# lkeegan/blockCG

Hardware: AMD Instinct MI355X
Metric: SBCGrQ lattice-site iterations/sec (iterations/sec x global volume), fp64 (higher is better)
Workload: dtype f64; 1 GPU; SBCGrQ V=64x64x64x64 (64x64x64x64 per GPU), m=16, 4 shifts, mass=0.001, fixed-work (eps=0); m=16, transport=none, half_volume_solves=False, memory_ladder_rung=whole tmp

## Files before the change

### blockcg_amd/csrc/capi_context.hip

```cpp
#include "capi_internal.hpp"

namespace bcg_impl {

std::string g_create_error;

void resolve_profile(bcg_context* c) {
  for (auto& kv : c->prof) {
    for (auto& pr : kv.second.pending) {
      float ms = 0.f;
      if (hipEventElapsedTime(&ms, pr.first, pr.second) == hipSuccess) {
        kv.second.ms += ms;
        kv.second.count += 1;
      }
      c->event_pool.push_back(pr.first);
      c->event_pool.push_back(pr.second);
    }
    kv.second.pending.clear();
  }
}

int stream_sync(bcg_context* c) {
  HIP_TRY(c, hipStreamSynchronize(c->stream));
  c->mat_in_flight = 0;
  if (c->profiling) resolve_profile(c);
// ... 272 lines not shown

}

using namespace bcg_impl;

extern "C" {

const char* bcg_last_error(const bcg_context* ctx) { return ctx ? ctx->err.c_str() : g_create_error.c_str(); }

int bcg_context_create(bcg_context** out, int device, void* stream, int ndim, const int* global_dims, const int* grid,
                       const int* coords) {
  if (!out || !global_dims || ndim < 1 || ndim > 4) {
    g_create_error = "bcg_context_create: bad arguments";
    return BCG_ERR_INVALID;
  }
  int ndev = 0;
  if (hipGetDeviceCount(&ndev) != hipSuccess || ndev <= 0 || device < 0 || device >= ndev) {
    g_create_error = "bcg_context_create: no usable HIP device (this library has no CPU fallback)";
    return BCG_ERR_NO_DEVICE;
  }
  hipDeviceProp_t prop;
  if (hipGetDeviceProperties(&prop, device) != hipSuccess) {
    g_create_error = "bcg_context_create: hipGetDeviceProperties failed";
    return BCG_ERR_NO_DEVICE;
  }
  if (std::strncmp(prop.gcnArchName, "gfx950", 6) != 0) {
    g_create_error = std::string("bcg_context_create: device is not gfx950 (MI355X): ") + prop.gcnArchName;
    return BCG_ERR_NO_DEVICE;
  }
  if (hipSetDevice(device) != hipSuccess) {
    g_create_error = "bcg_context_create: hipSetDevice failed";
    return BCG_ERR_HIP;
  }
  bcg_context* c = new bcg_context();
  c->device = device;
  c->ndim = ndim;
  int64_t V = 1;
  int64_t ghost = 0;
  for (int mu = 0; mu < 4; ++mu) {
    c->gdims[mu] = mu < ndim ? global_dims[mu] : 1;
    c->grid[mu] = (mu < ndim && grid) ? grid[mu] : 1;
    c->coords[mu] = (mu < ndim && coords) ? coords[mu] : 0;
    if (c->gdims[mu] < 1 || c->grid[mu] < 1 || c->gdims[mu] % c->grid[mu] != 0 || c->coords[mu] < 0 ||
        c->coords[mu] >= c->grid[mu]) {
      g_create_error = "bcg_context_create: lattice extents must be positive multiples of the process grid";
      delete c;
      return BCG_ERR_INVALID;
    }
    c->lat.L[mu] = c->gdims[mu] / c->grid[mu];
    c->lat.origin[mu] = c->coords[mu] * c->lat.L[mu];
    c->lat.split[mu] = c->grid[mu] > 1 ? 1 : 0;
    c->lat.stride[mu] = V;
    V *= c->lat.L[mu];
    if (c->lat.split[mu]) c->distributed = true;
  }
  c->lat.ndim = ndim;
  c->lat.V = V;
  for (int mu = 0; mu < 4; ++mu) {
    c->lat.face_sites[mu] = V / c->lat.L[mu];
    c->lat.ghost_off[mu][0] = c->lat.ghost_off[mu][1] = 0;
    if (c->lat.split[mu]) {
      c->lat.ghost_off[mu][0] = ghost;
      c->lat.ghost_off[mu][1] = ghost + c->lat.face_sites[mu];
      ghost += 2 * c->lat.face_sites[mu];
    }
  }
  c->ghost_sites = ghost;
  if (const char* e = std::getenv("BCG_ROW_BLOCKS_B")) c->row_blocks_B = std::atoi(e);
  if (const char* e = std::getenv("BCG_ROW_BLOCKS_C")) c->row_blocks_C = std::atoi(e);
  if (const char* e = std::getenv("BCG_ROW_BATCHED")) c->row_batched = std::atoi(e) != 0;
  if (const char* e = std::getenv("BCG_HOP_FACTORED")) c->hop_factored = std::atoi(e) != 0;
  if (const char* e = std::getenv("BCG_HOP_WALK")) c->hop_tune.patch_walk = std::atoi(e) != 0;
  if (const char* e = std::getenv("BCG_HOP_BLOCKS")) c->hop_tune.blocks = std::atoi(e);
  if (const char* e = std::getenv("BCG_HOP_BLOCKS_OVERLAP")) c->hop_tune.blocks_overlap = std::atoi(e);
  if (const char* e = std::getenv("BCG_HOP_SUPER")) c->hop_tune.super_patch = std::atoi(e);
  if (const char* e = std::getenv("BCG_HOP_SYNC")) c->hop_tune.sync.window = std::atoi(e);
  if (const char* e = std::getenv("BCG_HOP_SYNC_LIMIT")) c->hop_tune.sync.limit_ticks = std::atoi(e);
  if (const char* e = std::getenv("BCG_HOP_COLUMN")) c->hop_tune.sync.column_walk = std::atoi(e) != 0;
  if (const char* e = std::getenv("BCG_HOP_BUNDLE")) c->hop_tune.sync.bundle_walk = std::atoi(e);
  if (const char* e = std::getenv("BCG_HOP_BUNDLE_SYNC")) c->hop_tune.sync.bundle_window = std::atoi(e);
  if (const char* e = std::getenv("BCG_LAZY_Q")) c->lazy_q = std::atoi(e);
  if (const char* e = std::getenv("BCG_PAIR_SHIFTS")) c->pair_shifts = std::atoi(e);
  if (const char* e = std::getenv("BCG_DEFER_X0")) c->defer_x0 = std::atoi(e) != 0;
  if (const char* e = std::getenv("BCG_DEBUG_X0_COND_LIMIT")) c->x0_cond_limit = std::atof(e);
  if (const char* e = std::getenv("BCG_RING_CHUNK")) c->ring_chunk_override = std::atoi(e);
  if (const char* e = std::getenv("BCG_DEBUG_FIELD_BUDGET")) c->debug_field_budget = static_cast<size_t>(std::atoll(e));
  if (const char* e = std::getenv("BCG_DEBUG_FAIL_ITER")) c->debug_fail_iter = std::atoi(e);
  if (const char* e = std::getenv("BCG_RING_OVERLAP")) c->ring_overlap = std::atoi(e) != 0;
  if (const char* e = std::getenv("BCG_HALF_CHUNK_FORCE")) c->half_chunk_force = std::atoi(e) != 0;
  if (const char* e = std::getenv("BCG_HALF_CHUNK")) c->half_chunk_override = std::atoi(e);
  if (const char* e = std::getenv("BCG_FORCE_TILE_CLASSES")) c->force_tile_classes = std::atoi(e) != 0;
  if (const char* e = std::getenv("BCG_HOP_PATCH")) std::sscanf(e, "%d,%d,%d", &c->hop_tune.patch[0], &c->hop_tune.patch[1], &c->hop_tune.patch[2]);
  if (stream) {
    c->stream = static_cast<hipStream_t>(stream);
  } else {
    if (hipStreamCreateWithFlags(&c->stream, hipStreamNonBlocking) != hipSuccess) {
      g_create_error = "bcg_context_create: hipStreamCreate failed";
      delete c;
      return BCG_ERR_HIP;
    }
    c->own_stream = true;
  }
  *out = c;
  return BCG_OK;
}

int bcg_context_destroy(bcg_context* c) {
  DeviceScope on_device(c);
  if (!c) return BCG_OK;
  (void)hipSetDevice(c->device);
  (void)hipStreamSynchronize(c->stream);
  for (auto& kv : c->tmp_field) {
    (void)hipFree(kv.second->base);
    delete kv.second;
  }
  for (auto& kv : c->tmp_ring_buf)
    if (kv.second) (void)hipFree(kv.second);
  for (auto& kv : c->boundary_tiles)
    if (kv.second.first) (void)hipFree(kv.second.first);
  if (c->halo_send) (void)hipFree(c->halo_send);
  if (c->halo_recv) (void)hipFree(c->halo_recv);
  if (c->halo_save) (void)hipFree(c->halo_save);
  if (c->partials) (void)hipFree(c->partials);
  if (c->hop_tune.sync.counters) (void)hipFree(c->hop_tune.sync.counters);
  if (c->dev_mats) (void)hipFree(c->dev_mats);
  if (c->pin_mats) (void)hipHostFree(c->pin_mats);
  if (c->dev_gram) (void)hipFree(c->dev_gram);
  if (c->fold_tickets) (void)hipFree(c->fold_tickets);
  if (c->pin_gram) (void)hipHostFree(c->pin_gram);
  if (c->dev_basis) (void)hipFree(c->dev_basis);
  if (c->pin_basis) (void)hipHostFree(c->pin_basis);
  if (c->basis_uploaded) (void)hipEventDestroy(c->basis_uploaded);
  if (c->dev_rotate) (void)hipFree(c->dev_rotate);
  if (c->pin_rotate) (void)hipHostFree(c->pin_rotate);
  if (c->rotate_uploaded) (void)hipEventDestroy(c->rotate_uploaded);
  if (c->staging) (void)hipFree(c->staging);
  for (int k = 0; k < 2; ++k) {
    if (c->xfer_stream[k]) (void)hipStreamSynchronize(c->xfer_stream[k]);
    if (c->xfer_dev[k]) (void)hipFree(c->xfer_dev[k]);
    if (c->xfer_pin[k]) (void)hipHostFree(c->xfer_pin[k]);
    if (c->xfer_done[k]) (void)hipEventDestroy(c->xfer_done[k]);
    if (c->xfer_stream[k]) (void)hipStreamDestroy(c->xfer_stream[k]);
    c->xfer_dev[k] = nullptr;
    c->xfer_pin[k] = nullptr;
    c->xfer_done[k] = nullptr;
    c->xfer_stream[k] = nullptr;
  }
  for (auto& kv : c->prof)
    for (auto& pr : kv.second.pending) {
      (void)hipEventDestroy(pr.first);
      (void)hipEventDestroy(pr.second);
    }
  for (hipEvent_t ev : c->event_pool) (void)hipEventDestroy(ev);
  if (c->own_stream) (void)hipStreamDestroy(c->stream);
  delete c;
  return BCG_OK;
}

int bcg_context_set_comm(bcg_context* c, const bcg_comm* comm) {
  if (!c) return BCG_ERR_INVALID;
  if (comm) {
    c->comm = *comm;
    c->have_comm = true;
  } else {
    c->have_comm = false;
  }
// ... 391 lines not shown
```

### blockcg_amd/csrc/capi_solvers.hip

```cpp
#include "capi_internal.hpp"

namespace bcg_impl {

int phase_A(bcg_context* c, const bcg_gauge* g, double mass, double sigma0, bcg_field* T, const bcg_field* P, CMat& G) {
  int nb = 0;
  bool folded = false, self = false;
  BCG_TRY(apply_shifted(c, g, mass, sigma0, T, P, &nb, &folded, &self));
  if (nb > 0) {
    BCG_TRY(finish_gram(c, P->m, nb, G, true, folded));
    c->phaseA_gram_raw = CMat(P->m, c->pin_gram);
    if (self)
      for (int i = 0; i < P->m; ++i) G(i, i) = G(i, i).real();
    c->phaseA_gram = G;
    return BCG_OK;
  }
  BCG_TRY(gram(c, P, T, G));
  c->phaseA_gram = G;
  c->phaseA_gram_raw = CMat();
  return BCG_OK;
}

int rmul(bcg_context* c, bcg_field* y, const bcg_field* x, const CMat& M, double b, bcg::RmulMode mode, const char* name);
bool lazy_q_width(const bcg_context* c, int m) {
  return c->lazy_q && fast_rows(c, m) && fast_rmul(c, m) && (m == 8 || m == 16 || (m == 32 && c->lazy_q > 1));
}

int phase_B(bcg_context* c, bcg_field* Q, const bcg_field* T, const CMat& alpha, CMat& G2, const CMat* rinv_prev = nullptr,
            bcg_field* Qout = nullptr) {
  const int m = Q->m;
  if (!fast_rows(c, m)) {
    if (Qout) BCG_FAIL(c, BCG_ERR_INVALID, "phase B: a separate output needs the fused kernel");
    BCG_TRY(rmul(c, Q, T, -alpha, 0.0, bcg::RMUL_ADD, "block_axpy"));
    return gram(c, Q, Q, G2);
  }
  const CMat na = -alpha;
  const CMat* two[2] = {&na, rinv_prev};
  const double2* Md;
  BCG_TRY(upload_mats(c, m, two, rinv_prev ? 2 : 1, &Md));
  int nb;
  {
    ProfScope ps(c, "phaseB", row_bytes(Q, 3), product_flops(Q, rinv_prev ? 3 : 2));
    nb = bcg::launch_phaseB(c->stream, m, rows_of(Q), Q->d, T->d, Md, c->partials, c->row_blocks_B, c->row_batched,
                            bcg::GramFold{c->dev_gram, c->fold_tickets},
                            rinv_prev ? Md + static_cast<size_t>(m) * m : nullptr, Qout ? Qout->d : nullptr);
  }
  BCG_TRY(check_launch(c, "phaseB"));
  return finish_gram(c, m, nb, G2, true, true);
}

int trisolve(bcg_context* c, bcg_field* y, const CMat& R);
int phase_C(bcg_context* c, bcg_field* Q, const CMat& rho, bcg_field* const* X, bcg_field* const* P, int n,
            const std::vector<CMat>& A, const std::vector<CMat>& Bm, CMat* rinv_out = nullptr, bcg_field* Y = nullptr) {
  const int m = Q->m;
  if (!fast_rmul(c, m)) {
    BCG_TRY(trisolve(c, Q, rho));
    for (int s = 0; s < n; ++s) {
      BCG_TRY(rmul(c, Y ? Y : X[s], P[s], A[s], 0.0, bcg::RMUL_ADD, "block_axpy"));
      BCG_TRY(rmul(c, P[s], Q, Bm[s], 1.0, bcg::RMUL_XPAY, "block_xpay"));
    }
    return BCG_OK;
  }
  const CMat Rinv = bcg::upper_triangular_inverse(rho);
  if (rinv_out) *rinv_out = Rinv;
  for (int s0 = 0, first = 1, per = 0; first || s0 < n; s0 += per, first = 0) {
    per = bcg::phaseC_max_shifts(m, first != 0);
    const int ns = std::min(per, n - s0);
    std::vector<const CMat*> mats;
    mats.push_back(&Rinv);
    double2* Xp[8];
    double2* Pp[8];
    for (int k = 0; k < ns; ++k) {
      mats.push_back(&A[s0 + k]);
      mats.push_back(&Bm[s0 + k]);
      Xp[k] = Y ? nullptr : X[s0 + k]->d;
      Pp[k] = P[s0 + k]->d;
    }
    const double2* Md;
    BCG_TRY(upload_mats(c, m, mats.data(), static_cast<int>(mats.size()), &Md));
    {
      ProfScope ps(c, Y ? "phaseC_sum" : "phaseC", row_bytes(Q, (first && !rinv_out ? 2 : 1) + (Y ? 2 * ns + (ns > 0 ? 2 : 0) : 4 * ns)),
                   product_flops(Q, (rinv_out || first ? 1 : 0) + 2 * ns));
      bcg::launch_phaseC(c->stream, m, rows_of(Q), Q->d, Xp, Pp, ns, Md, rinv_out ? 2 : first, c->row_blocks_C, Y ? Y->d : nullptr);
    }
    BCG_TRY(check_launch(c, "phaseC"));
  }
  return BCG_OK;
}

bool x0_may_wait(const bcg_context* c, int m) {
  return c->defer_x0 && lazy_q_width(c, m) && (m == 8 || m == 16) && !capacity_path(c, m);
}
int pair_shifts_depth(const bcg_context* c, int m, int n_shifts) {
  if (c->pair_shifts < 2 || !fast_rows(c, m) || !fast_rmul(c, m)) return 1;
  if (!lazy_q_width(c, m) && m != 32) return 1;
  if (m == 32 && lazy_q_width(c, m)) return 1;
  int d = std::min(c->pair_shifts, capacity_path(c, m) ? 2 : 4);
  while (d >= 2 && !bcg::phaseC_multi_fits(m, d, n_shifts)) --d;
  if (n_shifts < 2 && (d < 3 || !x0_may_wait(c, m))) return 1;
  return d;
}

struct DeferredIteration {
  bcg_field* Q = nullptr;
  CMat rinv;
  int n_active = 0;
  std::vector<CMat> A, B;
  bool x0_deferred = false;
  CMat A0, R0;
  bool x0_backward = false;
};

struct DeferredX0 {
  std::vector<CMat> mats;
};
DeferredX0 compose_x0(const std::vector<DeferredIteration>& pend) {
  DeferredX0 out;
  const int n = static_cast<int>(pend.size());
  if (n == 0 || !pend[0].x0_deferred || pend[0].x0_backward) return out;
  const int m = pend[0].A0.dim();
  for (int k = -1; k + 1 < n; ++k) {
    CMat sum(m), chain = CMat::identity(m);
    for (int i = k + 1; i < n; ++i) {
      sum = sum + chain * pend[i].A0;
      chain = chain * pend[i].R0;
    }
    out.mats.push_back(sum);
  }
  return out;
}

int phase_C_multi(bcg_context* c, const std::vector<DeferredIteration>& pend, bcg_field* Qnew, const CMat& rho_new,
                  bcg_field* const* X, bcg_field* const* P, const CMat& A0, const CMat& B0, int n_active_new,
                  const std::vector<CMat>& Anew, const std::vector<CMat>& Bnew, CMat* rinv_out, bool lazy,
                  const CMat* flush_rinv = nullptr, const bcg_field* p0_first = nullptr, bcg_field* Y = nullptr) {
  const int m = Qnew->m, ns = static_cast<int>(pend.size()) + 1;
  const CMat rinv_new = flush_rinv ? *flush_rinv : (lazy ? bcg::upper_triangular_inverse(rho_new) : CMat());
  const double2* Qd[4];
  for (int j = 0; j + 1 < ns; ++j) Qd[j] = pend[j].Q->d;
  Qd[ns - 1] = Qnew->d;
  struct Entry {
    int shift, first, last;
    std::vector<const CMat*> mats;
  };
  std::vector<Entry> entries;
  if (flush_rinv) {
  } else if (lazy) {
    entries.push_back(Entry{0, ns - 1, ns, {&A0, &B0}});
  } else {
    const std::vector<CMat> a0(1, A0), b0(1, B0);
    BCG_TRY(phase_C(c, Qnew, rho_new, X, P, 1, a0, b0, nullptr, Y));
  }
  const int n_first = ns > 1 ? pend[0].n_active : n_active_new;
  for (int s = 1; s < n_first; ++s) {
    Entry e{s, 0, 0, {}};
    for (int j = 0; j < ns; ++j) {
      const bool on = s < (j + 1 < ns ? pend[j].n_active : n_active_new);
      if (!on) break;
      e.mats.push_back(j + 1 < ns ? &pend[j].A[s] : &Anew[s]);
      e.mats.push_back(j + 1 < ns ? &pend[j].B[s] : &Bnew[s]);
      ++e.last;
    }
    entries.push_back(e);
  }
  DeferredX0 x0 = (p0_first && lazy && !flush_rinv) ? compose_x0(pend) : DeferredX0();
  CMat A0_back;
  if (!p0_first && lazy && !flush_rinv && ns == 2 && pend[0].x0_deferred && pend[0].x0_backward) {
    const CMat M = pend[0].rinv.adjoint() * pend[0].A0;
    A0_back = A0 + M;
    entries[0].mats[0] = &A0_back;
    x0.mats.push_back(CMat(m));
    x0.mats.push_back(-M);
  }
  const int xacc = static_cast<int>(x0.mats.size());
  if (xacc > 0) {
    for (const CMat& M : x0.mats) entries[0].mats.push_back(&M);
  }
  static const char* const names[5] = {"", "", "phaseC_multi2", "phaseC_multi3", "phaseC_multi4"};
  static const char* const sum_names[5] = {"", "", "phaseC_multi2_sum", "phaseC_multi3_sum", "phaseC_multi4_sum"};
  for (size_t e0 = 0; e0 < entries.size();) {
    const bool with_x0 = xacc > 0 && e0 == 0;
    int n = 0;
    for (int room = bcg::phaseC_multi_capacity(m) - (lazy ? ns : 0); e0 + n < entries.size() && n < 8; ++n) {
      room -= static_cast<int>(entries[e0 + n].mats.size());
      if (room < 0) break;
    }
    if (n == 0) BCG_FAIL(c, BCG_ERR_UNSUPPORTED, "phase C: the matrices of one entry do not fit a launch");
    std::vector<const CMat*> mats;
    if (lazy) {
      for (int j = 0; j + 1 < ns; ++j) mats.push_back(&pend[j].rinv);
      mats.push_back(&rinv_new);
    }
    double2* Xp[8];
    double2* Pp[8];
    int first[8], last[8];
    double products = lazy ? ns : 0;
    for (int k = 0; k < n; ++k) {
      const Entry& e = entries[e0 + k];
      Xp[k] = Y ? nullptr : X[e.shift]->d;
      Pp[k] = P[e.shift]->d;
      first[k] = e.first;
      last[k] = e.last;
      mats.insert(mats.end(), e.mats.begin(), e.mats.end());
      products += static_cast<double>(e.mats.size());
    }
    const double2* Md;
    BCG_TRY(upload_mats(c, m, mats.data(), static_cast<int>(mats.size()), &Md));
    {
      const double2* const p1 = (with_x0 && p0_first) ? p0_first->d : nullptr;
      ProfScope ps(c, Y ? sum_names[ns] : names[ns], row_bytes(Qnew, ns + (Y ? 2 * n + 2 : 4 * n) + (p1 ? 1 : 0)),
                   product_flops(Qnew, products - ((with_x0 && !p1) ? 1 : 0)));
      bcg::launch_phaseC_multi(c->stream, m, rows_of(Qnew), ns, Qd, Xp, Pp, n, first, last, Md, c->row_blocks_C, lazy,
                               with_x0 ? xacc : 0, p1, Y ? Y->d : nullptr);
    }
    BCG_TRY(check_launch(c, "phaseC_multi"));
    e0 += n;
  }
  if (rinv_out) *rinv_out = rinv_new;
  return BCG_OK;
}

int thin_qr(bcg_context* c, bcg_field* y, CMat& R) {
  CMat G;
  BCG_TRY(gram(c, y, y, G));
  if (!G.all_finite()) BCG_FAIL(c, BCG_ERR_NUMERIC, "thinQR: Gram matrix is not finite");
  if (!bcg::cholesky_upper(G, R)) BCG_FAIL(c, BCG_ERR_NUMERIC, "thinQR: Gram matrix is not positive definite");
  return trisolve(c, y, R);
}

double max_ratio(const std::vector<double>& num, const std::vector<double>& den) {
  double r = 0.0;
  for (size_t i = 0; i < num.size(); ++i) r = std::max(r, num[i] / den[i]);
  return r;
}

}

using namespace bcg_impl;

namespace {

int real_dot(bcg_context* c, const bcg_field* a, const bcg_field* b, double& out) {
  CMat G;
  BCG_TRY(gram(c, a, b, G, false));
  out = G(0, 0).real();
  return BCG_OK;
}

struct FieldPool {
  bcg_context* c;
  std::vector<bcg_field*> f;
  int parity = -1;
  explicit FieldPool(bcg_context* ctx) : c(ctx) {}
  ~FieldPool() {
    for (bcg_field* p : f) bcg_field_destroy(p);
  }
  int make(int m, bcg_field** out, const bcg_field* init = nullptr) {
    bcg_field* p = nullptr;
    const int par = init ? init->parity : parity;
    if (par >= 0) BCG_TRY(bcg_field_create_half(c, m, par, &p));
    else BCG_TRY(bcg_field_create(c, m, &p));
    f.push_back(p);
    if (init) BCG_TRY(bcg_field_copy(p, init));
    *out = p;
    return BCG_OK;
  }
};

}

extern "C" {

int bcg_true_residuals(bcg_context* c, const bcg_gauge* g, double mass, bcg_field* const* X, const bcg_field* B,
                       int n_shifts, const double* sigma, double* res_out) {
  DeviceScope on_device(c);
  if (!c || !g || !X || !B || !sigma || !res_out || n_shifts < 1 || g->ctx != c || B->ctx != c) return BCG_ERR_INVALID;
  const int m = B->m;
  FieldPool pool(c);
  pool.parity = B->parity;
  bcg_field* AX = nullptr;
  CMat b2, r2;
  BCG_TRY(gram(c, B, B, b2));
  for (int s = 0; s < n_shifts; ++s) {
    if (!same_shape(X[s], B)) return BCG_ERR_INVALID;
    bcg::HopLaunchPlan fused;
    if (m == 16 && B->parity < 0 && fast_hop(c, m) && !capacity_path(c, m)) {
      BCG_TRY(ensure_scratch(c));
      fused = plan_stencil(c, c->lat, c->hop_tune, {m, bcg::HOP_RESID, true});
    }
    if (fused.form != bcg::HOP_FORM_NONE) {
      bcg_field* tmp;
      BCG_TRY(get_tmp(c, m, &tmp));
      BCG_TRY(hop(c, g, tmp, X[s], bcg::HOP_PLAIN, nullptr, 0.0));
      BCG_TRY(halo_field(c, tmp));
      int nb;
      {
        ProfScope ps(c, "hop_residual", alg_bytes(c, m, 3, 1));
        nb = bcg::hop_launch(c->stream, fused, g->U, g->Ughost, tmp->d, c->halo_recv, const_cast<double2*>(B->d), X[s]->d,
                             mass * mass + sigma[s], c->partials);
      }
      BCG_TRY(check_launch(c, "hop_residual"));
      BCG_TRY(finish_gram(c, m, nb, r2, true));
      for (int i = 0; i < m; ++i) res_out[s * m + i] = std::sqrt(r2(i, i).real() / b2(i, i).real());
      continue;
    }
    if (!AX) BCG_TRY(pool.make(m, &AX));
    BCG_TRY(apply_shifted(c, g, mass, sigma[s], AX, X[s]));
    BCG_TRY(axpby(c, AX, 1.0, B, -1.0, "axpby"));
    BCG_TRY(gram(c, AX, AX, r2));
    for (int i = 0; i < m; ++i) res_out[s * m + i] = std::sqrt(r2(i, i).real() / b2(i, i).real());
  }
  return BCG_OK;
}

int bcg_cg_solve(bcg_context* c, const bcg_gauge* g, double mass, bcg_field* x, const bcg_field* b, double eps,
                 int max_iterations, int* iterations_out) {
// ... 121 lines not shown
    BCG_TRY(rmul(c, X, P, alpha, 0.0, bcg::RMUL_ADD, "block_axpy"));
    BCG_TRY(rmul(c, P, R, beta, 1.0, bcg::RMUL_XPAY, "block_xpay"));
    residual = 0.0;
    for (int i = 0; i < m; ++i) residual = std::max(residual, std::sqrt(r2(i, i).real()) / norm0[i]);
  }
  BCG_TRY(stream_sync(c));
  if (iterations_out) *iterations_out = iter;
  return BCG_OK;
}

int bcg_bcgrq_solve(bcg_context* c, const bcg_gauge* g, double mass, bcg_field* X, const bcg_field* B, double eps,
                    int max_iterations, int* iterations_out) {
  DeviceScope on_device(c);
  const double zero = 0.0;
  bcg_field* Xs[1] = {X};
  return bcg_sbcgrq_solve(c, g, mass, Xs, const_cast<bcg_field*>(B), 1, &zero, eps, 0.0, max_iterations, 0, iterations_out,
                          nullptr, nullptr);
}

double bcg_sbcgrq_bytes_per_iteration(const bcg_context* c, int m, int n_shifts) {
  if (!c) return 0.0;
  const double s = 48.0 * m, gl = 144.0 * c->ndim;
  return static_cast<double>(c->lat.V) * ((14.0 + 4.0 * (n_shifts - 1)) * s + 2.0 * gl);
}

}

struct bcg_sbcgrq_state {
  bcg_context* c = nullptr;
  const bcg_gauge* g = nullptr;
  double mass = 0.0;
  int m = 0, n_shifts = 0;
  std::vector<double> sigma;
  double eps = 0.0, eps_shifts = 0.0;
  std::vector<bcg_field*> X;
  bcg_field* Y = nullptr;
  std::vector<double> residue;
  bcg_field* B = nullptr;
  bcg_field* T = nullptr;
  bcg_field* Q = nullptr;
  std::vector<bcg_field*> P;
  int n_unconverged = 0;
  CMat alpha, rho, delta, alpha_inv, alpha_inv_old, rho_old;
  std::vector<CMat> alpha_s, beta_s;
  std::vector<double> b_norm;
  double residual = 1.0;
  int iter = 0;
  CMat q_rinv;
  bool q_lazy = false;
  std::vector<DeferredIteration> pending;
  std::vector<bcg_field*> Qfree;
  int depth = 1;
  bool defer_x0 = false;
  bcg_field* P0_spare = nullptr;
  bcg_field* P0_first = nullptr;
  bool x0_backward = false;
  bool failed = false;
};

namespace {

void sbcgrq_release(bcg_sbcgrq_state* st) {
  if (st->T && st->T != st->B) bcg_field_destroy(st->T);
  if (st->Q && st->Q != st->B) bcg_field_destroy(st->Q);
  for (bcg_field* q : st->Qfree)
    if (q != st->B) bcg_field_destroy(q);
  for (const DeferredIteration& d : st->pending)
    if (d.Q != st->B && d.Q != st->Q) bcg_field_destroy(d.Q);
  st->Qfree.clear();
  st->pending.clear();
  if (st->P0_spare) bcg_field_destroy(st->P0_spare);
  if (st->P0_first) bcg_field_destroy(st->P0_first);
  st->P0_spare = st->P0_first = nullptr;
  for (bcg_field* p : st->P)
    if (p) bcg_field_destroy(p);
  st->T = st->Q = nullptr;
  st->P.clear();
}

int sbcgrq_iteration(bcg_sbcgrq_state* st, bcg_sbcgrq_trace* trace, bool more_follow) {
  bcg_context* c = st->c;
  const int m = st->m, n_shifts = st->n_shifts;
  const std::vector<double>& sigma = st->sigma;
  const CMat Identity = CMat::identity(m);
  ++st->iter;
  st->alpha_inv_old = st->alpha_inv;
  BCG_TRY(phase_A(c, st->g, st->mass, sigma[0], st->T, st->P[0], st->alpha_inv));
  if (!st->alpha_inv.all_finite()) BCG_FAIL(c, BCG_ERR_NUMERIC, "SBCGrQ: P^dagger A P is not finite");
  st->alpha = bcg::inverse_full_pivot(st->alpha_inv);
  const CMat alpha_delta = st->Y ? st->residue[0] * (st->alpha * st->delta) : st->alpha * st->delta;
  CMat G2;
  if (!st->pending.empty()) {
    const bool over_T = st->Qfree.empty();
    bcg_field* out = over_T ? st->T : st->Qfree.back();
    BCG_TRY(phase_B(c, st->Q, st->T, st->alpha, G2, st->q_lazy ? &st->q_rinv : nullptr, out));
    if (over_T) st->T = nullptr;
    else st->Qfree.pop_back();
    st->Q = out;
  } else {
    BCG_TRY(phase_B(c, st->Q, st->T, st->alpha, G2, st->q_lazy ? &st->q_rinv : nullptr));
  }
  st->rho_old = st->rho;
  if (c->debug_fail_iter > 0 && st->iter == c->debug_fail_iter) G2(0, 0) = cd(std::nan(""), 0.0);
  if (!G2.all_finite()) BCG_FAIL(c, BCG_ERR_NUMERIC, "thinQR: Gram matrix is not finite");
  if (!bcg::cholesky_upper(G2, st->rho)) BCG_FAIL(c, BCG_ERR_NUMERIC, "thinQR: Gram matrix is not positive definite");
  st->delta = st->rho * st->delta;
  st->residual = max_ratio(st->delta.row_norms(), st->b_norm);

  const bool tracing = trace && trace->recorded < trace->capacity;
  double* tm = nullptr;
  double* tr = nullptr;
  const size_t mm2 = static_cast<size_t>(m) * m * 2;
  if (tracing) {
    tm = trace->mats ? trace->mats + static_cast<size_t>(trace->recorded) * (3 + 2 * n_shifts) * mm2 : nullptr;
    tr = trace->res ? trace->res + static_cast<size_t>(trace->recorded) * (1 + n_shifts) : nullptr;
    if (tm) {
      std::memset(tm, 0, sizeof(double) * (3 + 2 * n_shifts) * mm2);
      st->alpha.store(tm);
      st->rho.store(tm + mm2);
      st->delta.store(tm + 2 * mm2);
    }
    if (tr) {
      tr[0] = st->residual;
      for (int s = 0; s < n_shifts; ++s) tr[1 + s] = -1.0;
    }
  }
  const CMat rho_dag = st->rho.adjoint();
  std::vector<CMat> Acoef(1, alpha_delta), Bcoef(1, rho_dag);
  std::vector<bcg_field*> Xa(1, st->X[0]), Pa(1, st->P[0]);
  std::vector<CMat> A_by_shift(n_shifts), B_by_shift(n_shifts);
  const int n_active = st->n_unconverged;
  for (int s = n_active - 1; s > 0; --s) {
    const CMat beta_s_inv = Identity + (sigma[s] - sigma[0]) * st->alpha +
                            st->alpha * st->rho_old * st->alpha_inv_old * (Identity - st->beta_s[s]) *
                                st->rho_old.adjoint();
    st->beta_s[s] = bcg::inverse_full_pivot(beta_s_inv);
    st->alpha_s[s] = st->beta_s[s] * st->alpha * st->rho_old * st->alpha_inv_old * st->alpha_s[s];
    const double residual_shift = max_ratio((st->rho * st->alpha_inv * st->alpha_s[s]).row_norms(), st->b_norm);
    Acoef.push_back(st->Y ? st->residue[s] * st->alpha_s[s] : st->alpha_s[s]);
    Bcoef.push_back(st->beta_s[s] * rho_dag);
    A_by_shift[s] = Acoef.back();
    B_by_shift[s] = Bcoef.back();
    Xa.push_back(st->X[s]);
    Pa.push_back(st->P[s]);
    if (tm) {
      st->alpha_s[s].store(tm + (3 + s) * mm2);
      st->beta_s[s].store(tm + (3 + n_shifts + s) * mm2);
    }
    if (tr) tr[1 + s] = residual_shift;
    if (residual_shift < st->eps_shifts) --st->n_unconverged;
  }
  const bool lazy = lazy_q_width(c, m);
  const bool next_certain = more_follow && st->residual > st->eps;
  const bool group_open = static_cast<int>(st->pending.size()) + 1 < st->depth && next_certain;
  bool x0_waits = group_open && st->defer_x0 && lazy &&
                  (st->pending.empty() ? st->P0_spare != nullptr : st->pending[0].x0_deferred);
  bool x0_backward = false;
  if (group_open && !x0_waits && st->x0_backward && lazy && st->depth == 2 && st->pending.empty() && n_active >= 2) {
    const CMat rinv = bcg::upper_triangular_inverse(st->rho);
    double f2 = 0.0, g2 = 0.0;
    for (int i = 0; i < m; ++i)
      for (int j = 0; j < m; ++j) {
        f2 += std::norm(st->rho(i, j));
        g2 += std::norm(rinv(i, j));
      }
    x0_backward = x0_waits = std::sqrt(f2 * g2) <= c->x0_cond_limit * m;
  }
  if (group_open && (n_active >= 2 || (x0_waits && st->depth >= 3))) {
    DeferredIteration d;
    if (x0_waits) {
      st->q_rinv = bcg::upper_triangular_inverse(st->rho);
      const CMat* two[2] = {&st->q_rinv, &rho_dag};
      const double2* Md;
      BCG_TRY(upload_mats(c, m, two, 2, &Md));
      bcg_field* const out = (st->pending.empty() && !x0_backward) ? st->P0_spare : st->P[0];
      {
        ProfScope ps(c, "phaseC_p0", row_bytes(st->Q, 3), product_flops(st->Q, 2));
        bcg::launch_phaseC_p0(c->stream, m, rows_of(st->Q), st->Q->d, st->P[0]->d, out->d, Md, c->row_blocks_C, c->row_batched);
      }
      BCG_TRY(check_launch(c, "phaseC_p0"));
      if (st->pending.empty() && !x0_backward) {
        st->P0_first = st->P[0];
        st->P[0] = st->P0_spare;
        st->P0_spare = nullptr;
      }
      d.x0_deferred = true;
      d.x0_backward = x0_backward;
      d.A0 = alpha_delta;
      d.R0 = rho_dag;
    } else {
      BCG_TRY(phase_C(c, st->Q, st->rho, Xa.data(), Pa.data(), 1, Acoef, Bcoef, lazy ? &st->q_rinv : nullptr, st->Y));
    }
    d.Q = st->Q;
    d.rinv = st->q_rinv;
    d.n_active = n_active;
    d.A = A_by_shift;
    d.B = B_by_shift;
    st->pending.push_back(d);
  } else if (!st->pending.empty()) {
    std::vector<DeferredIteration> pend;
    pend.swap(st->pending);
    const int rc = phase_C_multi(c, pend, st->Q, st->rho, st->X.data(), st->P.data(), alpha_delta, rho_dag, n_active,
                                 A_by_shift, B_by_shift, lazy ? &st->q_rinv : nullptr, lazy, nullptr, st->P0_first, st->Y);
    for (const DeferredIteration& d : pend) {
      if (!st->T) st->T = d.Q;
      else st->Qfree.push_back(d.Q);
    }
    if (st->P0_first) {
      st->P0_spare = st->P0_first;
      st->P0_first = nullptr;
    }
    BCG_TRY(rc);
  } else {
    BCG_TRY(phase_C(c, st->Q, st->rho, Xa.data(), Pa.data(), static_cast<int>(Xa.size()), Acoef, Bcoef,
                    lazy ? &st->q_rinv : nullptr, st->Y));
  }
  st->q_lazy = lazy;
  if (tracing) trace->recorded += 1;
  return BCG_OK;
}

int sbcgrq_flush_pending(bcg_sbcgrq_state* st) {
  if (st->pending.empty()) return BCG_OK;
  bcg_context* c = st->c;
  const int m = st->m;
  std::vector<DeferredIteration> pend;
  pend.swap(st->pending);
  const DeferredIteration last = pend.back();
  pend.pop_back();
  const bool lazy = lazy_q_width(c, m);
  int rc = BCG_OK;
  if (pend.empty()) {
    for (int s0 = 1; s0 < last.n_active && rc == BCG_OK;) {
      const int ns = std::min(bcg::phaseC_max_shifts(m, false), last.n_active - s0);
      const CMat unused = CMat::identity(m);
      std::vector<const CMat*> mats(1, lazy ? &last.rinv : &unused);
      double2* Xp[8];
      double2* Pp[8];
      for (int k = 0; k < ns; ++k) {
        mats.push_back(&last.A[s0 + k]);
        mats.push_back(&last.B[s0 + k]);
        Xp[k] = st->Y ? nullptr : st->X[s0 + k]->d;
        Pp[k] = st->P[s0 + k]->d;
      }
      const double2* Md;
      rc = upload_mats(c, m, mats.data(), static_cast<int>(mats.size()), &Md);
      if (rc != BCG_OK) break;
      bcg::launch_phaseC(c->stream, m, rows_of(last.Q), last.Q->d, Xp, Pp, ns, Md, lazy ? 2 : 0, c->row_blocks_C,
                         st->Y ? st->Y->d : nullptr);
      rc = check_launch(c, "phaseC");
      s0 += ns;
    }
  } else {
    const CMat none;
    rc = phase_C_multi(c, pend, last.Q, none, st->X.data(), st->P.data(), none, none, last.n_active, last.A, last.B, nullptr,
                       lazy, &last.rinv, nullptr, st->Y);
  }
  pend.push_back(last);
  bcg_field* const X0 = st->Y ? st->Y : st->X[0];
  if (rc == BCG_OK && pend[0].x0_deferred && pend[0].x0_backward) {
    const CMat M = pend[0].rinv.adjoint() * pend[0].A0;
    rc = rmul(c, X0, st->P[0], M, 0.0, bcg::RMUL_ADD, "block_axpy");
    if (rc == BCG_OK) rc = rmul(c, X0, pend[0].Q, -(pend[0].rinv * M), 0.0, bcg::RMUL_ADD, "block_axpy");
  } else if (rc == BCG_OK && st->P0_first && pend[0].x0_deferred) {
    const DeferredX0 x0 = compose_x0(pend);
    rc = rmul(c, X0, st->P0_first, x0.mats[0], 0.0, bcg::RMUL_ADD, "block_axpy");
    for (size_t k = 0; k + 1 < x0.mats.size() && rc == BCG_OK; ++k)
      rc = rmul(c, X0, pend[k].Q, pend[k].rinv * x0.mats[k + 1], 0.0, bcg::RMUL_ADD, "block_axpy");
  }
  if (st->P0_first) {
    st->P0_spare = st->P0_first;
    st->P0_first = nullptr;
  }
  for (const DeferredIteration& d : pend) {
    if (d.Q == st->Q || d.Q == st->T) continue;
    if (!st->T) st->T = d.Q;
    else st->Qfree.push_back(d.Q);
  }
  if (rc == BCG_OK) rc = stream_sync(c);
  return rc;
}

int sbcgrq_begin(bcg_context* c, const bcg_gauge* g, double mass, bcg_field* const* X, bcg_field* B, int n_shifts,
                 const double* sigma, double eps, double eps_shifts, int consume_B, bcg_sbcgrq_state** out, bcg_field* Y,
                 const double* residue, double c0) {
  if (!c || !g || !(X || Y) || !B || !sigma || !out || n_shifts < 1 || g->ctx != c || B->ctx != c) return BCG_ERR_INVALID;
  const int m = B->m;
  if (Y) {
    if (!same_shape(Y, B) || Y == B) BCG_FAIL(c, BCG_ERR_INVALID, "SBCGrQ_sum: Y must be a field of B's width and parity, distinct from B");
    if (!residue) BCG_FAIL(c, BCG_ERR_INVALID, "SBCGrQ_sum: one residue per shift is needed");
    if (!std::isfinite(c0)) BCG_FAIL(c, BCG_ERR_INVALID, "SBCGrQ_sum: c0 is not finite");
    for (int s = 0; s < n_shifts; ++s)
      if (!std::isfinite(residue[s])) BCG_FAIL(c, BCG_ERR_INVALID, "SBCGrQ_sum: a residue is not finite");
  } else {
    for (int s = 0; s < n_shifts; ++s)
      if (!same_shape(X[s], B) || X[s] == B) BCG_FAIL(c, BCG_ERR_INVALID, "SBCGrQ: X[s] must be distinct fields of B's width");
// ... 175 lines not shown
```

### blockcg_amd/csrc/context.hpp

```cpp
#pragma once
#include <hip/hip_runtime.h>

#include <map>
#include <string>
#include <vector>

#include "../../include/blockcg_hip.h"
#include "kernels.hpp"
#include "kernels_mfma.hpp"
#include "small_matrix.hpp"

struct bcg_field {
  bcg_context* ctx;
  int m;
  double2* d;
  void* base;
  int parity = -1;
  int64_t sites = 0;
};

struct bcg_gauge {
  bcg_context* ctx;
  double2* U;
  double2* Ughost;
  bool ghost_valid;
};

namespace bcg {

struct ProfEntry {
  double ms = 0.0;
  long count = 0;
  double bytes = 0.0;
  double flops = 0.0;
  std::vector<std::pair<hipEvent_t, hipEvent_t>> pending;
};

}

struct bcg_context {
  int device = 0;
  hipStream_t stream = nullptr;
  bool own_stream = false;
  int ndim = 1;
  int gdims[4] = {1, 1, 1, 1};
  int grid[4] = {1, 1, 1, 1};
  int coords[4] = {0, 0, 0, 0};
  bcg::LatticeDev lat{};
  int64_t ghost_sites = 0;
  bool distributed = false;
  bcg_comm comm{};
  bool have_comm = false;
  bool force_generic = false;
  bool force_tile_classes = false;
  int row_blocks_B = 1024, row_blocks_C = 1024;
  bool row_batched = true;
  bcg::HopTuning hop_tune;
  bcg::CMat phaseA_gram;
  bcg::CMat phaseA_gram_raw;
  bool hop_factored = true;

  std::map<int, bcg_field*> tmp_field;
  int tmp_ring = 0;
  std::map<int, double2*> tmp_ring_buf;
  std::map<int, std::pair<int*, int>> boundary_tiles;
  double2* halo_send = nullptr;
  double2* halo_recv = nullptr;
  size_t halo_bytes = 0;
  void* halo_save = nullptr;
  size_t halo_save_bytes = 0;
  int lazy_q = 1;
  int pair_shifts = 4;
  bool defer_x0 = true;
  double x0_cond_limit = 64.0;
  size_t debug_field_budget = 0;
  size_t field_bytes_live = 0;
  int debug_fail_iter = 0;
  int ring_chunk_override = 0;
  bool half_chunk_force = false;
  int half_chunk_override = 0;
  bool ring_overlap = true;
  double2* partials = nullptr;
  size_t partials_bytes = 0;
  double2* dev_mats = nullptr;
  double* pin_mats = nullptr;
  size_t mat_slot_bytes = 0;
  int mat_slots = 0, mat_next = 0, mat_in_flight = 0;
  unsigned* fold_tickets = nullptr;
  double2* dev_gram = nullptr;
  double* pin_gram = nullptr;
  double2* dev_basis = nullptr;
  double* pin_basis = nullptr;
  size_t basis_entries = 0;
  hipEvent_t basis_uploaded = nullptr;
  double2* dev_rotate = nullptr;
  double* pin_rotate = nullptr;
  hipEvent_t rotate_uploaded = nullptr;
  double2* staging = nullptr;
  size_t staging_bytes = 0;
  hipStream_t xfer_stream[2] = {nullptr, nullptr};
  hipEvent_t xfer_done[2] = {nullptr, nullptr};
  double2* xfer_dev[2] = {nullptr, nullptr};
  void* xfer_pin[2] = {nullptr, nullptr};
  size_t xfer_bytes = 0;

  bool profiling = false;
  std::map<std::string, bcg::ProfEntry> prof;
  std::vector<hipEvent_t> event_pool;
  std::string prof_json;

  mutable std::string err;
};
```

Measured before the change: 384.9 million site-iter/s.

## Overlap host shift-coefficient math with phase B kernel execution

Splits phase B into a launch step and a finish step, so host-side work runs while the GPU kernel executes before the Gram readback blocks. That work is the multi-shift beta/alpha recurrences that do not depend on the new rho, plus the deferred x0 composition. Rho-dependent parts (residuals, B coefficients) are moved to a later step. The aim is to hide CPU small-matrix inversions behind device time. It adds state-ordering complexity and is on by default, with an environment toggle to disable it.

```diff
diff --git a/blockcg_amd/csrc/capi_context.hip b/blockcg_amd/csrc/capi_context.hip
--- a/blockcg_amd/csrc/capi_context.hip
+++ b/blockcg_amd/csrc/capi_context.hip
@@ -378,6 +378,7 @@
   if (const char* e = std::getenv("BCG_LAZY_Q")) c->lazy_q = std::atoi(e);
   if (const char* e = std::getenv("BCG_PAIR_SHIFTS")) c->pair_shifts = std::atoi(e);
   if (const char* e = std::getenv("BCG_DEFER_X0")) c->defer_x0 = std::atoi(e) != 0;
+  if (const char* e = std::getenv("BCG_HOST_OVERLAP")) c->host_overlap = std::atoi(e) != 0;
   if (const char* e = std::getenv("BCG_DEBUG_X0_COND_LIMIT")) c->x0_cond_limit = std::atof(e);
   if (const char* e = std::getenv("BCG_RING_CHUNK")) c->ring_chunk_override = std::atoi(e);
   if (const char* e = std::getenv("BCG_DEBUG_FIELD_BUDGET")) c->debug_field_budget = static_cast<size_t>(std::atoll(e));
diff --git a/blockcg_amd/csrc/capi_solvers.hip b/blockcg_amd/csrc/capi_solvers.hip
--- a/blockcg_amd/csrc/capi_solvers.hip
+++ b/blockcg_amd/csrc/capi_solvers.hip
@@ -1,6 +1,9 @@
 #include "capi_internal.hpp"
+#include "shift_coeffs.hpp"
 
 namespace bcg_impl {
+
+using bcg::max_ratio;
 
 int phase_A(bcg_context* c, const bcg_gauge* g, double mass, double sigma0, bcg_field* T, const bcg_field* P, CMat& G) {
   int nb = 0;
@@ -25,27 +28,29 @@
   return c->lazy_q && fast_rows(c, m) && fast_rmul(c, m) && (m == 8 || m == 16 || (m == 32 && c->lazy_q > 1));
 }
 
-int phase_B(bcg_context* c, bcg_field* Q, const bcg_field* T, const CMat& alpha, CMat& G2, const CMat* rinv_prev = nullptr,
-            bcg_field* Qout = nullptr) {
+int phase_B_launch(bcg_context* c, bcg_field* Q, const bcg_field* T, const CMat& alpha, int* nb, const CMat* rinv_prev = nullptr,
+                   bcg_field* Qout = nullptr) {
   const int m = Q->m;
   if (!fast_rows(c, m)) {
     if (Qout) BCG_FAIL(c, BCG_ERR_INVALID, "phase B: a separate output needs the fused kernel");
-    BCG_TRY(rmul(c, Q, T, -alpha, 0.0, bcg::RMUL_ADD, "block_axpy"));
-    return gram(c, Q, Q, G2);
+    *nb = -1;
+    return rmul(c, Q, T, -alpha, 0.0, bcg::RMUL_ADD, "block_axpy");
   }
   const CMat na = -alpha;
   const CMat* two[2] = {&na, rinv_prev};
   const double2* Md;
   BCG_TRY(upload_mats(c, m, two, rinv_prev ? 2 : 1, &Md));
-  int nb;
   {
     ProfScope ps(c, "phaseB", row_bytes(Q, 3), product_flops(Q, rinv_prev ? 3 : 2));
-    nb = bcg::launch_phaseB(c->stream, m, rows_of(Q), Q->d, T->d, Md, c->partials, c->row_blocks_B, c->row_batched,
-                            bcg::GramFold{c->dev_gram, c->fold_tickets},
-                            rinv_prev ? Md + static_cast<size_t>(m) * m : nullptr, Qout ? Qout->d : nullptr);
-  }
-  BCG_TRY(check_launch(c, "phaseB"));
-  return finish_gram(c, m, nb, G2, true, true);
+    *nb = bcg::launch_phaseB(c->stream, m, rows_of(Q), Q->d, T->d, Md, c->partials, c->row_blocks_B, c->row_batched,
+                             bcg::GramFold{c->dev_gram, c->fold_tickets},
+                             rinv_prev ? Md + static_cast<size_t>(m) * m : nullptr, Qout ? Qout->d : nullptr);
+  }
+  return check_launch(c, "phaseB");
+}
+int phase_B_finish(bcg_context* c, const bcg_field* Q, int nb, CMat& G2) {
+  if (nb < 0) return gram(c, Q, Q, G2);
+  return finish_gram(c, Q->m, nb, G2, true, true);
 }
 
 int trisolve(bcg_context* c, bcg_field* y, const CMat& R);
@@ -132,7 +137,8 @@
 int phase_C_multi(bcg_context* c, const std::vector<DeferredIteration>& pend, bcg_field* Qnew, const CMat& rho_new,
                   bcg_field* const* X, bcg_field* const* P, const CMat& A0, const CMat& B0, int n_active_new,
                   const std::vector<CMat>& Anew, const std::vector<CMat>& Bnew, CMat* rinv_out, bool lazy,
-                  const CMat* flush_rinv = nullptr, const bcg_field* p0_first = nullptr, bcg_field* Y = nullptr) {
+                  const CMat* flush_rinv = nullptr, const bcg_field* p0_first = nullptr, bcg_field* Y = nullptr,
+                  const DeferredX0* x0_pre = nullptr) {
   const int m = Qnew->m, ns = static_cast<int>(pend.size()) + 1;
   const CMat rinv_new = flush_rinv ? *flush_rinv : (lazy ? bcg::upper_triangular_inverse(rho_new) : CMat());
   const double2* Qd[4];
@@ -162,7 +168,7 @@
     }
     entries.push_back(e);
   }
-  DeferredX0 x0 = (p0_first && lazy && !flush_rinv) ? compose_x0(pend) : DeferredX0();
+  DeferredX0 x0 = (p0_first && lazy && !flush_rinv) ? (x0_pre ? *x0_pre : compose_x0(pend)) : DeferredX0();
   CMat A0_back;
   if (!p0_first && lazy && !flush_rinv && ns == 2 && pend[0].x0_deferred && pend[0].x0_backward) {
     const CMat M = pend[0].rinv.adjoint() * pend[0].A0;
@@ -225,12 +231,6 @@
   if (!G.all_finite()) BCG_FAIL(c, BCG_ERR_NUMERIC, "thinQR: Gram matrix is not finite");
   if (!bcg::cholesky_upper(G, R)) BCG_FAIL(c, BCG_ERR_NUMERIC, "thinQR: Gram matrix is not positive definite");
   return trisolve(c, y, R);
-}
-
-double max_ratio(const std::vector<double>& num, const std::vector<double>& den) {
-  double r = 0.0;
-  for (size_t i = 0; i < num.size(); ++i) r = std::max(r, num[i] / den[i]);
-  return r;
 }
 
 }
@@ -518,28 +518,50 @@
   bcg_context* c = st->c;
   const int m = st->m, n_shifts = st->n_shifts;
   const std::vector<double>& sigma = st->sigma;
-  const CMat Identity = CMat::identity(m);
   ++st->iter;
   st->alpha_inv_old = st->alpha_inv;
   BCG_TRY(phase_A(c, st->g, st->mass, sigma[0], st->T, st->P[0], st->alpha_inv));
   if (!st->alpha_inv.all_finite()) BCG_FAIL(c, BCG_ERR_NUMERIC, "SBCGrQ: P^dagger A P is not finite");
   st->alpha = bcg::inverse_full_pivot(st->alpha_inv);
-  const CMat alpha_delta = st->Y ? st->residue[0] * (st->alpha * st->delta) : st->alpha * st->delta;
+  const int n_active = st->n_unconverged;
+  const bool overlap = c->host_overlap;
+  bcg::ShiftCoeffs sc;
+  CMat alpha_delta;
+  DeferredX0 x0_pre;
+  bool have_x0_pre = false;
+  const auto before_rho = [&]() {
+    alpha_delta = st->Y ? st->residue[0] * (st->alpha * st->delta) : st->alpha * st->delta;
+    bcg::shift_coeffs_early(sc, n_active, sigma, st->alpha, st->rho, st->alpha_inv_old, st->beta_s, st->alpha_s,
+                            st->Y ? st->residue.data() : nullptr);
+  };
   CMat G2;
+  int nb = 0;
+  bcg_field* Qout = nullptr;
+  bool over_T = false;
   if (!st->pending.empty()) {
-    const bool over_T = st->Qfree.empty();
-    bcg_field* out = over_T ? st->T : st->Qfree.back();
-    BCG_TRY(phase_B(c, st->Q, st->T, st->alpha, G2, st->q_lazy ? &st->q_rinv : nullptr, out));
+    over_T = st->Qfree.empty();
+    Qout = over_T ? st->T : st->Qfree.back();
+  }
+  BCG_TRY(phase_B_launch(c, st->Q, st->T, st->alpha, &nb, st->q_lazy ? &st->q_rinv : nullptr, Qout));
+  if (overlap) {
+    before_rho();
+    if (!st->pending.empty() && st->P0_first && (static_cast<int>(st->pending.size()) + 1 >= st->depth || !more_follow)) {
+      x0_pre = compose_x0(st->pending);
+      have_x0_pre = true;
+    }
+  }
+  BCG_TRY(phase_B_finish(c, Qout ? Qout : st->Q, nb, G2));
+  if (Qout) {
     if (over_T) st->T = nullptr;
     else st->Qfree.pop_back();
-    st->Q = out;
-  } else {
-    BCG_TRY(phase_B(c, st->Q, st->T, st->alpha, G2, st->q_lazy ? &st->q_rinv : nullptr));
-  }
+    st->Q = Qout;
+  }
+  if (!overlap) before_rho();
   st->rho_old = st->rho;
   if (c->debug_fail_iter > 0 && st->iter == c->debug_fail_iter) G2(0, 0) = cd(std::nan(""), 0.0);
   if (!G2.all_finite()) BCG_FAIL(c, BCG_ERR_NUMERIC, "thinQR: Gram matrix is not finite");
   if (!bcg::cholesky_upper(G2, st->rho)) BCG_FAIL(c, BCG_ERR_NUMERIC, "thinQR: Gram matrix is not positive definite");
+  bcg::shift_coeffs_commit(sc, st->beta_s, st->alpha_s);
   st->delta = st->rho * st->delta;
   st->residual = max_ratio(st->delta.row_norms(), st->b_norm);
 
@@ -562,30 +584,12 @@
     }
   }
   const CMat rho_dag = st->rho.adjoint();
-  std::vector<CMat> Acoef(1, alpha_delta), Bcoef(1, rho_dag);
-  std::vector<bcg_field*> Xa(1, st->X[0]), Pa(1, st->P[0]);
-  std::vector<CMat> A_by_shift(n_shifts), B_by_shift(n_shifts);
-  const int n_active = st->n_unconverged;
-  for (int s = n_active - 1; s > 0; --s) {
-    const CMat beta_s_inv = Identity + (sigma[s] - sigma[0]) * st->alpha +
-                            st->alpha * st->rho_old * st->alpha_inv_old * (Identity - st->beta_s[s]) *
-                                st->rho_old.adjoint();
-    st->beta_s[s] = bcg::inverse_full_pivot(beta_s_inv);
-    st->alpha_s[s] = st->beta_s[s] * st->alpha * st->rho_old * st->alpha_inv_old * st->alpha_s[s];
-    const double residual_shift = max_ratio((st->rho * st->alpha_inv * st->alpha_s[s]).row_norms(), st->b_norm);
-    Acoef.push_back(st->Y ? st->residue[s] * st->alpha_s[s] : st->alpha_s[s]);
-    Bcoef.push_back(st->beta_s[s] * rho_dag);
-    A_by_shift[s] = Acoef.back();
-    B_by_shift[s] = Bcoef.back();
-    Xa.push_back(st->X[s]);
-    Pa.push_back(st->P[s]);
-    if (tm) {
-      st->alpha_s[s].store(tm + (3 + s) * mm2);
-      st->beta_s[s].store(tm + (3 + n_shifts + s) * mm2);
-    }
-    if (tr) tr[1 + s] = residual_shift;
-    if (residual_shift < st->eps_shifts) --st->n_unconverged;
-  }
+  bool late_done = false;
+  const auto after_rho = [&]() {
+    bcg::shift_coeffs_late(sc, st->rho, st->alpha_inv, rho_dag, st->b_norm, st->eps_shifts, st->n_unconverged, tm, tr);
+    late_done = true;
+  };
+  if (!overlap) after_rho();
   const bool lazy = lazy_q_width(c, m);
   const bool next_certain = more_follow && st->residual > st->eps;
   const bool group_open = static_cast<int>(st->pending.size()) + 1 < st->depth && next_certain;
@@ -625,19 +629,23 @@
       d.A0 = alpha_delta;
       d.R0 = rho_dag;
     } else {
-      BCG_TRY(phase_C(c, st->Q, st->rho, Xa.data(), Pa.data(), 1, Acoef, Bcoef, lazy ? &st->q_rinv : nullptr, st->Y));
-    }
+      const std::vector<CMat> a0(1, alpha_delta), b0(1, rho_dag);
+      BCG_TRY(phase_C(c, st->Q, st->rho, st->X.data(), st->P.data(), 1, a0, b0, lazy ? &st->q_rinv : nullptr, st->Y));
+    }
+    if (!late_done) after_rho();
     d.Q = st->Q;
     d.rinv = st->q_rinv;
     d.n_active = n_active;
-    d.A = A_by_shift;
-    d.B = B_by_shift;
+    d.A = sc.A_by_shift;
+    d.B = sc.B_by_shift;
     st->pending.push_back(d);
   } else if (!st->pending.empty()) {
     std::vector<DeferredIteration> pend;
     pend.swap(st->pending);
+    if (!late_done) after_rho();
     const int rc = phase_C_multi(c, pend, st->Q, st->rho, st->X.data(), st->P.data(), alpha_delta, rho_dag, n_active,
-                                 A_by_shift, B_by_shift, lazy ? &st->q_rinv : nullptr, lazy, nullptr, st->P0_first, st->Y);
+                                 sc.A_by_shift, sc.B_by_shift, lazy ? &st->q_rinv : nullptr, lazy, nullptr, st->P0_first, st->Y,
+                                 have_x0_pre ? &x0_pre : nullptr);
     for (const DeferredIteration& d : pend) {
       if (!st->T) st->T = d.Q;
       else st->Qfree.push_back(d.Q);
@@ -648,6 +656,15 @@
     }
     BCG_TRY(rc);
   } else {
+    if (!late_done) after_rho();
+    std::vector<CMat> Acoef(1, alpha_delta), Bcoef(1, rho_dag);
+    std::vector<bcg_field*> Xa(1, st->X[0]), Pa(1, st->P[0]);
+    for (int s = n_active - 1; s > 0; --s) {
+      Acoef.push_back(sc.A_by_shift[s]);
+      Bcoef.push_back(sc.B_by_shift[s]);
+      Xa.push_back(st->X[s]);
+      Pa.push_back(st->P[s]);
+    }
     BCG_TRY(phase_C(c, st->Q, st->rho, Xa.data(), Pa.data(), static_cast<int>(Xa.size()), Acoef, Bcoef,
                     lazy ? &st->q_rinv : nullptr, st->Y));
   }
diff --git a/blockcg_amd/csrc/context.hpp b/blockcg_amd/csrc/context.hpp
--- a/blockcg_amd/csrc/context.hpp
+++ b/blockcg_amd/csrc/context.hpp
@@ -72,6 +72,7 @@
   int lazy_q = 1;
   int pair_shifts = 4;
   bool defer_x0 = true;
+  bool host_overlap = true;
   double x0_cond_limit = 64.0;
   size_t debug_field_budget = 0;
   size_t field_bytes_live = 0;
diff --git a/blockcg_amd/csrc/shift_coeffs.hpp b/blockcg_amd/csrc/shift_coeffs.hpp
--- /dev/null
+++ b/blockcg_amd/csrc/shift_coeffs.hpp
@@ -0,0 +1,70 @@
+#pragma once
+#include <algorithm>
+#include <cstddef>
+#include <vector>
+
+#include "small_matrix.hpp"
+
+namespace bcg {
+
+inline double max_ratio(const std::vector<double>& num, const std::vector<double>& den) {
+  double r = 0.0;
+  for (size_t i = 0; i < num.size(); ++i) r = std::max(r, num[i] / den[i]);
+  return r;
+}
+
+struct ShiftCoeffs {
+  int n_active = 0;
+  std::vector<CMat> beta_s, alpha_s;
+  std::vector<CMat> A_by_shift;
+  std::vector<CMat> B_by_shift;
+};
+
+inline void shift_coeffs_early(ShiftCoeffs& out, int n_active, const std::vector<double>& sigma, const CMat& alpha,
+                               const CMat& rho_old, const CMat& alpha_inv_old, const std::vector<CMat>& beta_s,
+                               const std::vector<CMat>& alpha_s, const double* residue) {
+  const int n_shifts = static_cast<int>(sigma.size());
+  out.n_active = n_active;
+  out.beta_s.assign(n_shifts, CMat());
+  out.alpha_s.assign(n_shifts, CMat());
+  out.A_by_shift.assign(n_shifts, CMat());
+  out.B_by_shift.assign(n_shifts, CMat());
+  if (n_active < 2) return;
+  const CMat Identity = CMat::identity(alpha.dim());
+  const CMat ara = alpha * rho_old * alpha_inv_old;
+  const CMat rho_old_dag = rho_old.adjoint();
+  for (int s = n_active - 1; s > 0; --s) {
+    const CMat beta_s_inv = Identity + (sigma[s] - sigma[0]) * alpha + ara * (Identity - beta_s[s]) * rho_old_dag;
+    out.beta_s[s] = inverse_full_pivot(beta_s_inv);
+    out.alpha_s[s] = out.beta_s[s] * alpha * rho_old * alpha_inv_old * alpha_s[s];
+    out.A_by_shift[s] = residue ? residue[s] * out.alpha_s[s] : out.alpha_s[s];
+  }
+}
+
+inline void shift_coeffs_commit(const ShiftCoeffs& sc, std::vector<CMat>& beta_s, std::vector<CMat>& alpha_s) {
+  for (int s = sc.n_active - 1; s > 0; --s) {
+    beta_s[s] = sc.beta_s[s];
+    alpha_s[s] = sc.alpha_s[s];
+  }
+}
+
+inline void shift_coeffs_late(ShiftCoeffs& sc, const CMat& rho, const CMat& alpha_inv, const CMat& rho_dag,
+                              const std::vector<double>& b_norm, double eps_shifts, int& n_unconverged, double* trace_mats,
+                              double* trace_res) {
+  if (sc.n_active < 2) return;
+  const int n_shifts = static_cast<int>(sc.beta_s.size());
+  const size_t mm2 = static_cast<size_t>(rho.dim()) * rho.dim() * 2;
+  const CMat rai = rho * alpha_inv;
+  for (int s = sc.n_active - 1; s > 0; --s) {
+    const double residual_shift = max_ratio((rai * sc.alpha_s[s]).row_norms(), b_norm);
+    sc.B_by_shift[s] = sc.beta_s[s] * rho_dag;
+    if (trace_mats) {
+      sc.alpha_s[s].store(trace_mats + (3 + s) * mm2);
+      sc.beta_s[s].store(trace_mats + (3 + n_shifts + s) * mm2);
+    }
+    if (trace_res) trace_res[1 + s] = residual_shift;
+    if (residual_shift < eps_shifts) --n_unconverged;
+  }
+}
+
+}
```

Measured after the change: 386.4 million site-iter/s, median of 6. No clear change (+0.4%).
